# nilsbore/gp_compressor

Hardware: AMD Instinct MI355X
Metric: patches/sec (compress+predict) (higher is better)
Workload: dtype f64; 1 GPU; C2 room scan: 8192 patches x 256 pts per GPU, RBF + Gaussian noise, dense Cholesky fit + predictive mean on the 20x20 grid (m=400); patches_per_gpu=8192, points_per_patch=256, grid_points=400, parallelism=1 GPU, kernel=dense_mfma_w1

## Files before the change

### gp_compressor_amd/csrc/dense_mfma_w1.hip

```cpp
#include <cstdio>
#include <cstdlib>
#include <type_traits>

#include "gpc_device.h"
#include "dense_internal.h"
#include "mfma_tile.h"

#define W1_NPAD_MAX 512
#define W1_C 4
#define W1_NDT 10
#define W1_NT_OF(npad) ((npad) / 16)
#define W1_TRI_OF(npad) (W1_NT_OF(npad) * (W1_NT_OF(npad) + 1) / 2)
#define W1_TILE(i, j) (((size_t)(i) * (size_t)((i) + 1) / 2 + (size_t)(j)) * MF_IMG)


struct W1Params {
    DenseArgs a;
    double c_exp;
    double pivot_tol;
    double cs, noise_u, sfp, a_out;
    double* ws;
    double* linvt;
    int export_factor;
    unsigned long long* stamps;
};
#define W1_NPH 12
#ifdef W1_STAMPS
#define W1_STAMP(ph)                                                                                                 \
    do {                                                                                                             \
        __builtin_amdgcn_sched_barrier(0);                                                                           \
        const unsigned long long t_now_ = __builtin_amdgcn_s_memtime();                                              \
        st_acc_[ph] += t_now_ - t_prev_;                                                                             \
        t_prev_ = t_now_;                                                                                            \
        __builtin_amdgcn_sched_barrier(0);                                                                           \
    } while (0)
#else
#define W1_STAMP(ph) do { } while (0)
#endif

#define W1_LDS_SYNC()                                                                                                \
    do {                                                                                                             \
        __builtin_amdgcn_fence(__ATOMIC_SEQ_CST, "wavefront");                                                       \
        __builtin_amdgcn_wave_barrier();                                                                             \
    } while (0)

template <int A, int B, typename F>
__device__ static __forceinline__ void w1_static_for(F&& f)
{
    if constexpr (A < B) {
        f(std::integral_constant<int, A>{});
        w1_static_for<A + 1, B>(f);
    }
}
__host__ __device__ constexpr int w1_stream_col(int q)
{
    int kk = 0;
    while ((kk + 1) * (kk + 2) / 2 <= q) ++kk;
    return kk;
}
#define W1_BW 20

__device__ static __forceinline__ d4 w1_mfma4_neg(d4 a, d4 b, d4 acc)
{
#pragma unroll
    for (int s = 0; s < 4; ++s) acc = __builtin_amdgcn_mfma_f64_16x16x4f64(a[s], b[s], acc, 0, 0, 1);
    return acc;
}
__device__ static __forceinline__ d4 w1_trsm(d4 lv, d4 src)
{
    const d4 z4 = d4{0.0, 0.0, 0.0, 0.0};
    d4 D = __builtin_amdgcn_mfma_f64_16x16x4f64(lv[0], src[0], z4, 0, 0, 0);
    D = __builtin_amdgcn_mfma_f64_16x16x4f64(lv[1], src[1], D, 0, 0, 0);
    D = __builtin_amdgcn_mfma_f64_16x16x4f64(lv[2], src[2], D, 0, 0, 0);
    return __builtin_amdgcn_mfma_f64_16x16x4f64(lv[3], src[3], D, 0, 0, 0);
}

template <int MODE, int CNT, bool DIAG>
__device__ static __forceinline__ void w1_gram_row(d4 (&v)[W1_C], const double* px0, const double* px1, const double* T, double sf, bool scale_sf,
                                                   double cexp, double noise, bool dbl, int n, int r, int c0, int lr, int lg)
{
    const int pi = MF_TS * r + lr;
    const double xi0 = px0[pi], xi1 = px1[pi];
#pragma unroll
    for (int t = 0; t < CNT; ++t) {
#pragma unroll
        for (int q = 0; q < 4; ++q) {
            const int pj = MF_TS * (c0 + t) + lg + 4 * q;
            const double d0 = xi0 - px0[pj], d1 = xi1 - px1[pj];
            const double sq = __builtin_fma(d0, d0, d1 * d1);
            v[t][q] = MODE == 0 ? gpc_exp_neg(cexp * sq, T) : gpc_expm_poly<MODE == 1 ? 7 : 5>(sq);
        }
    }
    if (scale_sf) {
#pragma unroll
        for (int t = 0; t < CNT; ++t)
#pragma unroll
            for (int q = 0; q < 4; ++q) v[t][q] *= sf;
    }
    if constexpr (DIAG) {
#pragma unroll
        for (int q = 0; q < 4; ++q) {
            double d = v[CNT - 1][q] + noise;
            if (dbl) d += noise;
            v[CNT - 1][q] = (lr == lg + 4 * q) ? d : v[CNT - 1][q];
        }
    }
    if (MF_TS * (r + 1) > n || MF_TS * (c0 + CNT) > n) {
#pragma unroll
        for (int t = 0; t < CNT; ++t) {
#pragma unroll
            for (int q = 0; q < 4; ++q) {
                const int pj = MF_TS * (c0 + t) + lg + 4 * q;
                if (pi >= n || pj >= n) v[t][q] = (pi == pj) ? 1.0 : 0.0;
            }
        }
    }
}

template <int W1_NPAD>
__global__ __launch_bounds__(64, 2) void dense_w1_kernel(W1Params g)
{
    constexpr int W1_NT = W1_NT_OF(W1_NPAD), W1_TRI = W1_TRI_OF(W1_NPAD);
    __shared__ __attribute__((aligned(16))) double T[GPC_EXP_TABLE_SIZE];
    __shared__ __attribute__((aligned(16))) double px0[W1_NPAD], px1[W1_NPAD], zv[W1_NPAD];
    __shared__ __attribute__((aligned(16))) double rsbuf[32], wsc[32];
    __shared__ __attribute__((aligned(16))) double LinvC[W1_C * MF_IMG];

    const DenseArgs& A = g.a;
    int lane = threadIdx.x;
    int lr = lane & 15, lg = lane >> 4;
#define W1_FRESH_LANE()                                                                                              \
    do {                                                                                                             \
        lane = mf_opaque(lane);                                                                                      \
        lr = lane & 15;                                                                                              \
        lg = lane >> 4;                                                                                              \
    } while (0)
    const int m = A.m;
    const double sf = A.prm.sigmaf_sq, cexp = g.c_exp;
    const bool dbl = A.prm.ref_double_noise != 0;
    const int patch = blockIdx.x;
    double* Lt = g.ws + (size_t)patch * W1_TRI * MF_IMG;
    double* LinvTg = g.linvt + (size_t)patch * W1_NT * MF_IMG;

    gpc_exp_table_init(T);
    {
        const int o = __builtin_amdgcn_readfirstlane(A.off[patch]);
        const int n = __builtin_amdgcn_readfirstlane(A.off[patch + 1]) - o;
        double* fs = A.f_star + (size_t)patch * m;
        __syncthreads();
        if (n <= 0 || n > W1_NPAD) {
            for (int p = lane; p < m; p += 64) fs[p] = (n == 0) ? 0.0 : __builtin_nan("");
            if (lane == 0 && A.status) A.status[patch] = (n == 0) ? GPC_STATUS_OK : GPC_STATUS_NAN;
            return;
        }
        const int nt = __builtin_amdgcn_readfirstlane((n + MF_TS - 1) / MF_TS);
#ifdef W1_STAMPS
        unsigned long long st_acc_[W1_NPH] = {};
        unsigned long long t_prev_ = __builtin_amdgcn_s_memtime();
#endif

        const double xo0 = A.x0[o], xo1 = A.x1[o];
        double qr0[W1_NPAD / 64], qr1[W1_NPAD / 64];
        double mn0 = xo0, mx0 = xo0, mn1 = xo1, mx1 = xo1;
#pragma unroll
        for (int u = 0; u < W1_NPAD / 64; ++u) {
            const int i = lane + 64 * u;
            const bool live = i < n;
            qr0[u] = live ? A.x0[o + i] : xo0;
            qr1[u] = live ? A.x1[o + i] : xo1;
            mn0 = __builtin_fmin(mn0, qr0[u]); mx0 = __builtin_fmax(mx0, qr0[u]);
            mn1 = __builtin_fmin(mn1, qr1[u]); mx1 = __builtin_fmax(mx1, qr1[u]);
            zv[i] = live ? A.y[o + i] : 0.0;
        }
#pragma unroll
        for (int o_ = 32; o_ > 0; o_ >>= 1) {
            mn0 = __builtin_fmin(mn0, __shfl_xor(mn0, o_, 64)); mx0 = __builtin_fmax(mx0, __shfl_xor(mx0, o_, 64));
            mn1 = __builtin_fmin(mn1, __shfl_xor(mn1, o_, 64)); mx1 = __builtin_fmax(mx1, __shfl_xor(mx1, o_, 64));
        }
        int mode_g, mode_p;
        {
            const bool nan_box = !((mx0 - mn0) + (mx1 - mn1) < __builtin_inf());
            const double rx = mx0 - mn0, ry = mx1 - mn1;
            const double tg = nan_box ? __builtin_inf() : -cexp * __builtin_fma(rx, rx, ry * ry);
            const double hb = 0.5 * A.grid_res;
            const double bx = hb + __builtin_fmax(__builtin_fabs(mn0), __builtin_fabs(mx0));
            const double by = hb + __builtin_fmax(__builtin_fabs(mn1), __builtin_fabs(mx1));
            const double bq = __builtin_fmax(bx, by);
            const double tp = nan_box ? __builtin_inf() : -cexp * (bq * bq);
            mode_g = __builtin_amdgcn_readfirstlane(tg <= GPC_EXP_TINY_MAX ? 2 : tg <= GPC_EXP_SMALL_MAX ? 1 : 0);
            mode_p = __builtin_amdgcn_readfirstlane(tp <= GPC_EXP_TINY_MAX ? 2 : tp <= GPC_EXP_SMALL_MAX ? 1 : 0);
            if (mode_g == 0) mode_p = 0;
        }
        const bool scaled = mode_g > 0;
        {
            const double cs = scaled ? g.cs : 1.0;
            const double co0 = scaled ? xo0 : 0.0, co1 = scaled ? xo1 : 0.0;
#pragma unroll
            for (int u = 0; u < W1_NPAD / 64; ++u) {
                const int i = lane + 64 * u;
                const bool live = i < n;
                px0[i] = live ? cs * (qr0[u] - co0) : 0.0;
                px1[i] = live ? cs * (qr1[u] - co1) : 0.0;
            }
        }
        const bool scale_sf = g.export_factor != 0;
        const double noise_u = g.noise_u, ptol = g.pivot_tol;
        W1_LDS_SYNC();
#define W1_GRAM_ROW(v, CNT, DIAG, r, c0)                                                                              \
    do {                                                                                                             \
        if (mode_g == 2) w1_gram_row<2, CNT, DIAG>(v, px0, px1, T, sf, scale_sf, cexp, noise_u, dbl, n, r, c0, lr, lg);   \
        else if (mode_g == 1) w1_gram_row<1, CNT, DIAG>(v, px0, px1, T, sf, scale_sf, cexp, noise_u, dbl, n, r, c0, lr, lg); \
        else w1_gram_row<0, CNT, DIAG>(v, px0, px1, T, sf, scale_sf, cexp, noise_u, dbl, n, r, c0, lr, lg);            \
    } while (0)

        auto bw_step = [&](auto P, const d4 img, d4& pa) __attribute__((always_inline)) {
            constexpr int q = decltype(P)::value;
            constexpr int kk = w1_stream_col(q), t = q - kk * (kk + 1) / 2;
            if (kk < nt) {
                const int k = nt - 1 - kk;
                if constexpr (t < kk) {
                    const double a_ = zv[MF_TS * (k + 1 + t) + lr];
                    pa += img * a_;
                } else {
                    d4 ub = d4{0.0, 0.0, 0.0, 0.0};
                    if constexpr (kk > 0) {
                        const double tot = mf_row_reduce4(pa, lr);
                        if ((lr & 3) == 0) wsc[lg + 4 * (lr >> 2)] = tot;
                        W1_LDS_SYNC();
                        if (lr == 0) {
#pragma unroll
                            for (int q4 = 0; q4 < 4; ++q4) ub[q4] = zv[MF_TS * k + lg + 4 * q4] - wsc[lg + 4 * q4];
                        }
                    } else {
                        if (lr == 0) {
#pragma unroll
                            for (int q4 = 0; q4 < 4; ++q4) ub[q4] = zv[MF_TS * k + lg + 4 * q4];
                        }
                    }
                    const d4 al = w1_trsm(img, ub);
                    W1_LDS_SYNC();
                    if (lr == 0) {
#pragma unroll
                        for (int r = 0; r < 4; ++r) zv[MF_TS * k + lg + 4 * r] = al[r];
                    }
                    W1_LDS_SYNC();
                    pa = d4{0.0, 0.0, 0.0, 0.0};
                }
            }
        };
        bool bad = false;
        W1_STAMP(0);
#define W1_BLOCK_ROW(bi, kb, nb)                                                                                     \
    do {                                                                                                             \
        if ((bi) < (nb)) {                                                                                           \
            d4 gv[W1_C];                                                                                             \
            W1_GRAM_ROW(gv, (bi) + 1, true, (kb) + (bi), (kb));                                                      \
            _Pragma("unroll") for (int bc = 0; bc <= (bi); ++bc) tacc[(bi) * ((bi) + 1) / 2 + bc] = gv[bc];           \
        } else {                                                                                                     \
            _Pragma("unroll") for (int bc = 0; bc <= (bi); ++bc) tacc[(bi) * ((bi) + 1) / 2 + bc] = d4{0.0, 0.0, 0.0, 0.0}; \
        }                                                                                                            \
    } while (0)
#define W1_BLOCK_INIT(kb, nb)                                                                                        \
    do {                                                                                                             \
        _Pragma("unroll") for (int i = 0; i < W1_C; ++i) part[i] = 0.0;                                              \
                                             \
        __builtin_amdgcn_sched_barrier(0);                                                                           \
        W1_BLOCK_ROW(3, kb, nb);                                                                                     \
        __builtin_amdgcn_sched_barrier(0);                                                                           \
        W1_BLOCK_ROW(2, kb, nb);                                                                                     \
        __builtin_amdgcn_sched_barrier(0);                                                                           \
        W1_BLOCK_ROW(1, kb, nb);                                                                                     \
        __builtin_amdgcn_sched_barrier(0);                                                                           \
        W1_BLOCK_ROW(0, kb, nb);                                                                                     \
        __builtin_amdgcn_sched_barrier(0);                                                                           \
    } while (0)
        W1_STAMP(1);
        for (int k = 0;; k += W1_C) {
            const int nc = min(W1_C, nt - k);
            const int kl = k - 1;
            const bool last_step = k + W1_C >= nt;
            (void)last_step;
            W1_FRESH_LANE();
            const double* rrow[W1_C];
#pragma unroll
            for (int i = 0; i < W1_C; ++i) rrow[i] = Lt + W1_TILE(k + min(i, nc - 1), 0);
            d4 tacc[W1_NDT];
            double part[W1_C];
            d4 op[2][W1_C];
#pragma unroll
            for (int i = 0; i < W1_C; ++i) op[0][i] = op[1][i] = d4{0.0, 0.0, 0.0, 0.0};
            if (k > 0) {
#pragma unroll
                for (int i = 0; i < W1_C; ++i) op[0][i] = mf_img_load(rrow[i], lane);
            }
            W1_BLOCK_INIT(k, nc);
            for (int j = 0; j < k; j += 2) {
#pragma unroll
                for (int h = 0; h < 2; ++h) {
                    const int jn = min(j + h + 1, kl);
#pragma unroll
                    for (int i = 0; i < W1_C; ++i) op[h ^ 1][i] = mf_img_load(rrow[i] + (size_t)jn * MF_IMG, lane);
#pragma unroll
                    for (int d = 0; d < W1_NDT; ++d) {
                        const int bi = d >= 6 ? 3 : d >= 3 ? 2 : d >= 1 ? 1 : 0, bc = d - bi * (bi + 1) / 2;
                        if (bi < nc) tacc[d] = w1_mfma4_neg(op[h][bc], op[h][bi], tacc[d]);
                    }
                    const double* zq = zv + MF_TS * (j + h) + lg;
                    const double z0 = zq[0], z1 = zq[4], z2 = zq[8], z3 = zq[12];
#pragma unroll
                    for (int c = 0; c < W1_C; ++c) part[c] += (op[h][c][0] * z0 + op[h][c][1] * z1) + (op[h][c][2] * z2 + op[h][c][3] * z3);
                }
            }
            W1_STAMP(2);
            W1_FRESH_LANE();
            d4 Lb[W1_C * (W1_C - 1) / 2];
#pragma unroll
            for (int q = 0; q < W1_C * (W1_C - 1) / 2; ++q) Lb[q] = d4{0.0, 0.0, 0.0, 0.0};
            bool ok = mf_diag_factor_c(tacc[0], rsbuf, LinvC, LinvTg + (size_t)k * MF_IMG, ptol, lane);
            W1_LDS_SYNC();
            if (g.export_factor) mf_img_store(Lt + W1_TILE(k, k), lane, mf_img_load(LinvC, lane));
#pragma unroll
            for (int i = 1; i < W1_C; ++i) {
                if (ok && i < nc) {
#pragma unroll
                    for (int c = 0; c < i; ++c) {
                        d4 Tt = tacc[i * (i + 1) / 2 + c];
#pragma unroll
                        for (int c2 = 0; c2 < c; ++c2) Tt = w1_mfma4_neg(Lb[c * (c - 1) / 2 + c2], Lb[i * (i - 1) / 2 + c2], Tt);
                        const d4 lvc = mf_img_load(LinvC + c * MF_IMG, mf_opaque(lane));
                        const d4 L = w1_trsm(lvc, Tt);
                        Lb[i * (i - 1) / 2 + c] = L;
                        mf_img_store(Lt + W1_TILE(k + i, k + c), lane, L);
                    }
                    d4 Dii = tacc[i * (i + 1) / 2 + i];
#pragma unroll
                    for (int c = 0; c < i; ++c) Dii = w1_mfma4_neg(Lb[i * (i - 1) / 2 + c], Lb[i * (i - 1) / 2 + c], Dii);
                    ok = mf_diag_factor_c(Dii, rsbuf, LinvC + i * MF_IMG, LinvTg + (size_t)(k + i) * MF_IMG, ptol, lane);
                    W1_LDS_SYNC();
                    if (g.export_factor) mf_img_store(Lt + W1_TILE(k + i, k + i), lane, mf_img_load(LinvC + i * MF_IMG, mf_opaque(lane)));
                }
            }
            if (!ok) { bad = true; break; }
            W1_STAMP(3);
            W1_FRESH_LANE();
#pragma unroll
            for (int c = 0; c < W1_C; ++c) {
                if (c < nc) {
                    const int pj = MF_TS * (k + c) + lr;
                    double pp = part[c];
#pragma unroll
                    for (int c2 = 0; c2 < c; ++c2) {
                        const d4 lb = Lb[c * (c - 1) / 2 + c2];
                        const double* zq = zv + MF_TS * (k + c2) + lg;
                        pp += (lb[0] * zq[0] + lb[1] * zq[4]) + (lb[2] * zq[8] + lb[3] * zq[12]);
                    }
                    pp += __shfl_xor(pp, 16, 64);
                    pp += __shfl_xor(pp, 32, 64);
                    const double yv = zv[pj];
                    W1_LDS_SYNC();
                    if (lg == 0) zv[pj] = yv - pp;
                    W1_LDS_SYNC();
                    const d4 lv = mf_img_load(LinvC + c * MF_IMG, mf_opaque(lane));
                    const double* tq = zv + MF_TS * (k + c) + lg;
                    double zz = (lv[0] * tq[0] + lv[1] * tq[4]) + (lv[2] * tq[8] + lv[3] * tq[12]);
                    zz += __shfl_xor(zz, 16, 64);
                    zz += __shfl_xor(zz, 32, 64);
                    W1_LDS_SYNC();
                    if (lg == 0) zv[pj] = zz;
                    W1_LDS_SYNC();
                }
            }
            W1_STAMP(4);
            const int rows_tot = nt - (k + nc);
            if (rows_tot == 0) {
                __syncthreads();
                break;
            }
            if (k > 0) __syncthreads();
            const int npass = (rows_tot + 3) / 4;
            const int klp = k - 1;
            if (k == 0) {
                for (int pi_ = 0; pi_ < npass; ++pi_) {
                    const int first_row0 = (pi_ + 1 < npass) ? 4 * (pi_ + 1) : 0;
                    const int np4 = min(4, rows_tot - first_row0);
                    W1_FRESH_LANE();
                    d4 cy[W1_C][4];
#pragma unroll
                    for (int t = 0; t < 4; ++t) {
                        const int r_ = W1_C + first_row0 + min(t, np4 - 1);
                        d4 gv[W1_C];
                        W1_GRAM_ROW(gv, 2, false, r_, 0);
                        cy[0][t] = gv[0]; cy[1][t] = gv[1];
                        __builtin_amdgcn_sched_barrier(0);
                        W1_GRAM_ROW(gv, 2, false, r_, 2);
                        cy[2][t] = gv[0]; cy[3][t] = gv[1];
                        __builtin_amdgcn_sched_barrier(0);
                    }
                    W1_STAMP(5);
#pragma unroll
                    for (int c = 0; c < W1_C; ++c) {
                        const d4 lv = mf_img_load(LinvC + c * MF_IMG, mf_opaque(lane));
#pragma unroll
                        for (int t = 0; t < 4; ++t) {
#pragma unroll
                            for (int c2 = 0; c2 < c; ++c2) cy[c][t] = w1_mfma4_neg(Lb[c * (c - 1) / 2 + c2], cy[c2][t], cy[c][t]);
                            cy[c][t] = w1_trsm(lv, cy[c][t]);
                            if (t < np4) mf_img_store(Lt + W1_TILE(W1_C + first_row0 + t, c), lane, cy[c][t]);
                        }
                    }
                    W1_STAMP(7);
                }
            }
            if (k > 0) {
                for (int pi_ = 0; pi_ < npass; ++pi_) {
                    const int first_row = (pi_ + 1 < npass) ? 4 * (pi_ + 1) : 0;
                    const int np4 = min(4, rows_tot - first_row);
                    W1_FRESH_LANE();
                    d4 cy[W1_C][4];
                    int rr[4];
                    const double* rw_[4];
#pragma unroll
                    for (int t = 0; t < 4; ++t) {
                        rr[t] = k + W1_C + first_row + min(t, np4 - 1);
                        rw_[t] = Lt + W1_TILE(rr[t], 0);
                    }
                    d4 A2[2][W1_C], B[4];
#pragma unroll
                    for (int c = 0; c < W1_C; ++c) A2[0][c] = mf_img_load(rrow[c], lane);
#pragma unroll
                    for (int t = 0; t < 4; ++t) B[t] = mf_img_load(rw_[t], lane);
#pragma unroll
                    for (int t = 0; t < 4; ++t) {
                        d4 gv[W1_C];
                        W1_GRAM_ROW(gv, 2, false, rr[t], k);
                        cy[0][t] = gv[0]; cy[1][t] = gv[1];
                        __builtin_amdgcn_sched_barrier(0);
                        W1_GRAM_ROW(gv, 2, false, rr[t], k + 2);
                        cy[2][t] = gv[0]; cy[3][t] = gv[1];
                        __builtin_amdgcn_sched_barrier(0);
                    }
                    W1_STAMP(5);
                    d4 Lq[W1_C * (W1_C - 1) / 2];
#define W1_PASS_J(st, jn, PREFETCH)                                                                                  \
    do {                                                                                                             \
                                      \
        if (PREFETCH) {                                                                                              \
            _Pragma("unroll") for (int c = 0; c < W1_C; ++c) A2[(st) ^ 1][c] = mf_img_load(rrow[c] + (size_t)(jn) * MF_IMG, lane); \
        }                                                                                                            \
        __builtin_amdgcn_sched_barrier(0);                                                                           \
        _Pragma("unroll") for (int t = 0; t < 4; ++t) {                                                              \
            _Pragma("unroll") for (int c = 0; c < W1_C; ++c) cy[c][t] = w1_mfma4_neg(A2[st][c], B[t], cy[c][t]);      \
            __builtin_amdgcn_sched_barrier(0);                                                                       \
            if (PREFETCH) B[t] = mf_img_load(rw_[t] + (size_t)(jn) * MF_IMG, lane);                                    \
            else {      \
                if (t < 3) Lq[t] = mf_img_load(Lt + W1_TILE(k + (t == 0 ? 1 : 2), k + (t == 2 ? 1 : 0)), lane);      \
                else {                                                                                               \
                    _Pragma("unroll") for (int c2 = 0; c2 < 3; ++c2) Lq[3 + c2] = mf_img_load(Lt + W1_TILE(k + 3, k + c2), lane); \
                }                                                                                                    \
            }                                                                                                        \
            __builtin_amdgcn_sched_barrier(0);                                                                       \
        }                                                                                                            \
    } while (0)
                    for (int j = 0; j + 2 < k; j += 2) {
                        W1_PASS_J(0, j + 1, true);
                        W1_PASS_J(1, j + 2, true);
                    }
                    W1_PASS_J(0, klp, true);
                    W1_PASS_J(1, klp, false);
#undef W1_PASS_J
                    W1_STAMP(6);
                    W1_FRESH_LANE();
#pragma unroll
                    for (int c = 0; c < W1_C; ++c) {
                        const d4 lv = mf_img_load(LinvC + c * MF_IMG, mf_opaque(lane));
#pragma unroll
                        for (int t = 0; t < 4; ++t) {
#pragma unroll
                            for (int c2 = 0; c2 < c; ++c2) cy[c][t] = w1_mfma4_neg(Lq[c * (c - 1) / 2 + c2], cy[c2][t], cy[c][t]);
                            cy[c][t] = w1_trsm(lv, cy[c][t]);
                            if (t < np4) mf_img_store(Lt + W1_TILE(rr[t], k + c), lane, cy[c][t]);
                        }
                    }
                    W1_STAMP(7);
                }
            }
            __syncthreads();
            W1_STAMP(8);
        }
#undef W1_BLOCK_INIT
#undef W1_BLOCK_ROW

        if (bad) {
            for (int p = lane; p < m; p += 64) fs[p] = __builtin_nan("");
            if (A.alpha_out)
                for (int i = lane; i < n; i += 64) A.alpha_out[o + i] = __builtin_nan("");
            if (lane == 0 && A.status) A.status[patch] = GPC_STATUS_NOT_SPD;
            return;
        }

        {
            W1_FRESH_LANE();
            constexpr int NP = W1_NPAD / MF_TS;
            constexpr int SLEN = NP * (NP + 1) / 2;
            d4 win[W1_BW];
            auto stream_addr = [&](auto P) __attribute__((always_inline)) -> const double* {
                constexpr int q = decltype(P)::value;
                constexpr int kk = w1_stream_col(q), t = q - kk * (kk + 1) / 2;
                const int kq = max(nt - 1 - kk, 0);
                const double* ad = (t < kk) ? Lt + W1_TILE(kq + 1 + t, kq) : LinvTg + (size_t)kq * MF_IMG;
                return kk < nt ? ad : Lt;
            };
            w1_static_for<0, W1_BW>([&](auto P) __attribute__((always_inline)) {
                constexpr int q = decltype(P)::value;
                win[q] = mf_img_load_nt(stream_addr(P), lane);
            });
            d4 pa = d4{0.0, 0.0, 0.0, 0.0};
            w1_static_for<0, SLEN>([&](auto P) __attribute__((always_inline)) {
                constexpr int q = decltype(P)::value;
                bw_step(P, win[q % W1_BW], pa);
                if constexpr (q + W1_BW < SLEN) {
                    win[q % W1_BW] = mf_img_load_nt(stream_addr(std::integral_constant<int, q + W1_BW>{}), lane);
                }
            });
        }
        W1_STAMP(9);
        double* av = zv;
        if (A.alpha_out)
            for (int i = lane; i < n; i += 64) A.alpha_out[o + i] = av[i] * g.a_out;

        W1_FRESH_LANE();
        if (m <= 0) {
        } else if (A.xs0 == nullptr && A.grid_sz <= 32) {
            const int sz = A.grid_sz;
            const double res = A.grid_res;
            d4 P[2][2];
#pragma unroll
            for (int mt = 0; mt < 2; ++mt)
#pragma unroll
                for (int nl = 0; nl < 2; ++nl) P[mt][nl] = d4{0.0, 0.0, 0.0, 0.0};
            double gqx[2], gqy[2];
            const double cs = scaled ? g.cs : 1.0, co0 = scaled ? A.x0[o] : 0.0, co1 = scaled ? A.x1[o] : 0.0;
            const double argc = scaled ? -1.0 : cexp, sfp = g.sfp;
#pragma unroll
            for (int h = 0; h < 2; ++h) {
                const double gq = res * (((double)(16 * h + lr) + 0.5) / (double)sz - 0.5);
                gqx[h] = cs * (gq - co0);
                gqy[h] = cs * (gq - co1);
            }
            auto predict_loop = [&](auto mode_tag) __attribute__((always_inline)) {
                constexpr int MP = decltype(mode_tag)::value;
                for (int ibase = 0; ibase < n; ibase += 32) {
#pragma unroll
                    for (int s = 0; s < 8; ++s) {
                        const int i = ibase + 4 * s + lg;
                        const int ic = min(i, W1_NPAD - 1);
                        const double al = (i < n) ? sfp * av[ic] : 0.0;
                        const double xi0 = px0[ic], xi1 = px1[ic];
                        double ea[2], eb[2];
#pragma unroll
                        for (int h = 0; h < 2; ++h) {
                            const double dy = gqy[h] - xi1, dx = gqx[h] - xi0;
                            if constexpr (MP == 0) {
                                ea[h] = gpc_exp_neg(argc * (dy * dy), T);
                                eb[h] = gpc_exp_neg(argc * (dx * dx), T) * al;
                            } else {
                                ea[h] = gpc_expm_poly<MP == 1 ? 7 : 5>(dy * dy);
                                eb[h] = gpc_expm_poly<MP == 1 ? 7 : 5>(dx * dx) * al;
                            }
                        }
#pragma unroll
                        for (int nl = 0; nl < 2; ++nl)
#pragma unroll
                            for (int mt = 0; mt < 2; ++mt)
                                P[mt][nl] = __builtin_amdgcn_mfma_f64_16x16x4f64(ea[mt], eb[nl], P[mt][nl], 0, 0, 0);
                    }
                }
            };
            if (mode_p == 2) predict_loop(std::integral_constant<int, 2>{});
            else if (mode_p == 1) predict_loop(std::integral_constant<int, 1>{});
            else predict_loop(std::integral_constant<int, 0>{});
#pragma unroll
            for (int mt = 0; mt < 2; ++mt)
#pragma unroll
                for (int nl = 0; nl < 2; ++nl)
#pragma unroll
                    for (int r = 0; r < 4; ++r) {
                        const int py = 16 * mt + lg + 4 * r, pxx = 16 * nl + lr;
                        if (py < sz && pxx < sz) fs[py * sz + pxx] = P[mt][nl][r];
                    }
        } else {
            const double cs = scaled ? g.cs : 1.0, co0 = scaled ? A.x0[o] : 0.0, co1 = scaled ? A.x1[o] : 0.0;
            const double argc = scaled ? -1.0 : cexp, sfp = g.sfp;
            for (int p = lane; p < m; p += 64) {
                double q0, q1;
                if (A.xs0) {
                    q0 = A.xs0[p];
                    q1 = A.xs1[p];
                } else {
                    const int gx = p % A.grid_sz, gy = p / A.grid_sz;
                    q0 = A.grid_res * (((double)gx + 0.5) / (double)A.grid_sz - 0.5);
                    q1 = A.grid_res * (((double)gy + 0.5) / (double)A.grid_sz - 0.5);
                }
                q0 = cs * (q0 - co0);
                q1 = cs * (q1 - co1);
                double s_ = 0.0;
                for (int i = 0; i < n; ++i) {
                    const double d0 = px0[i] - q0, d1 = px1[i] - q1;
                    s_ += gpc_exp_neg(argc * __builtin_fma(d0, d0, d1 * d1), T) * av[i];
                }
                fs[p] = sfp * s_;
            }
        }
        if (lane == 0 && A.status) A.status[patch] = GPC_STATUS_OK;
#ifdef W1_STAMPS
        W1_STAMP(10);
        if (g.stamps && lane == 0)
            for (int q_ = 0; q_ < W1_NPH; ++q_) atomicAdd(g.stamps + q_, st_acc_[q_]);
#endif
    }
}

static int w1_npad(const DenseArgs& a) { return a.n_max <= 256 ? 256 : W1_NPAD_MAX; }

bool dense_w1_supported(const DenseArgs& a)
{
    if (a.v_star) return a.n_max <= 256 && a.ny == 1 && !a.sel && a.xs0 != nullptr;
    return a.n_max <= W1_NPAD_MAX && a.ny == 1 && !a.sel;
}

#define W1_MAX_SLOTS 8192
static int w1_chunk(const DenseArgs& a, int cap_in)
{
    const char* e = getenv("GPC_W1_SLOTS");
    int cap = e && atoi(e) > 0 ? atoi(e) : W1_MAX_SLOTS;
    if (cap_in > 0 && cap_in < cap) cap = cap_in;
    return a.P < cap ? a.P : cap;
}

size_t dense_w1_ws_bytes(const gpc_ctx* ctx, const DenseArgs& a, int* grid_out, int cap)
{
    (void)ctx;
    const int grid = w1_chunk(a, cap);
    if (grid_out) *grid_out = grid;
    const int npad = w1_npad(a);
    return sizeof(double) * ((size_t)(W1_TRI_OF(npad) + W1_NT_OF(npad)) * MF_IMG * (size_t)grid + (a.v_star ? (size_t)a.n_total : 0));
}

int dense_w1_launch(gpc_ctx* ctx, const DenseSite& site, const DenseArgs& a_in, int grid)
{
    DenseArgs a = a_in;
    double* v_star = a.v_star;
    a.v_star = nullptr;
    W1Params g;
    g.c_exp = (double)(-0.5f) / a.prm.l_sq;
    g.ws = reinterpret_cast<double*>(dense_ws(ctx, site));
    const int npad = w1_npad(a);
    g.linvt = g.ws + (size_t)W1_TRI_OF(npad) * MF_IMG * (size_t)grid;
    g.export_factor = v_star ? 1 : 0;
    const double sf = a.prm.sigmaf_sq;
    const bool unit = !v_star;
    g.cs = sqrt(-g.c_exp);
    g.noise_u = unit ? a.prm.noise / sf : a.prm.noise;
    g.pivot_tol = GPC_PIVOT_RTOL * (unit ? 1.0 + a.prm.noise / sf : sf + a.prm.noise);
    g.sfp = unit ? 1.0 : sf;
    g.a_out = unit ? 1.0 / sf : 1.0;
    g.stamps = nullptr;
    if (v_star) {
        a.m = 0;
        if (!a.alpha_out) a.alpha_out = g.linvt + (size_t)W1_NT_OF(npad) * MF_IMG * (size_t)grid;
    }
    ctx->last_dense_kernel = v_star ? "dense_mfma_w1 + dense_variance" : npad == 256 ? "dense_mfma_w1" : "dense_mfma_w1_512";
#ifdef W1_STAMPS
    if (getenv("GPC_W1_STAMPS")) {
        GPC_HIP(ctx, hipMalloc(&g.stamps, sizeof(unsigned long long) * W1_NPH));
        GPC_HIP(ctx, hipMemsetAsync(g.stamps, 0, sizeof(unsigned long long) * W1_NPH, site.stream));
    }
#endif
    for (int base = 0; base < a.P; base += grid) {
        const int cnt = a.P - base < grid ? a.P - base : grid;
        g.a = a;
        g.a.P = cnt;
        g.a.off = a.off + base;
        g.a.f_star = a.f_star ? a.f_star + (size_t)base * a.ny * a_in.m : nullptr;
        g.a.status = a.status ? a.status + base : nullptr;
        if (npad == 256) hipLaunchKernelGGL((dense_w1_kernel<256>), dim3(cnt), dim3(64), 0, site.stream, g);
        else hipLaunchKernelGGL((dense_w1_kernel<W1_NPAD_MAX>), dim3(cnt), dim3(64), 0, site.stream, g);
        GPC_HIP(ctx, hipGetLastError());
        if (v_star) {
            DenseArgs av = g.a;
            av.m = a_in.m;
            const int rc = dense_variance_launch(ctx, site, av, W1_NT_OF(256), g.ws, a.alpha_out, v_star + (size_t)base * a_in.m);
            if (rc != GPC_OK) return rc;
        }
    }
#ifdef W1_STAMPS
    if (g.stamps) {
        unsigned long long h[W1_NPH];
        GPC_HIP(ctx, hipStreamSynchronize(site.stream));
        GPC_HIP(ctx, hipMemcpy(h, g.stamps, sizeof(h), hipMemcpyDeviceToHost));
        (void)hipFree(g.stamps);
        static const char* names[W1_NPH] = {"load", "sweep gram", "sweep loop", "chain", "forward", "pass gram", "pass loop", "pass trsm",
                                            "step fence", "backward", "predict", ""};
        unsigned long long tot = 0;
        for (int q = 0; q < W1_NPH; ++q) tot += h[q];
        fprintf(stderr, "[GPC_W1_STAMPS] mean s_memtime ticks per patch (total %.0f)\n", (double)tot / a.P);
        for (int q = 0; q < 11; ++q) fprintf(stderr, "  %-12s %9.0f  %5.1f %%\n", names[q], (double)h[q] / a.P, 100.0 * h[q] / tot);
    }
#endif
    return GPC_OK;
}
```

### gp_compressor_amd/csrc/mfma_tile.h

```cpp
#pragma once

#include "gpc_device.h"

typedef double d4 __attribute__((ext_vector_type(4)));
#define MF_TS 16

__device__ static __forceinline__ int mf_opaque(int v)
{
    asm volatile("" : "+v"(v));
    return v;
}

__device__ static __forceinline__ bool mf_wait_ge(unsigned lds_byte_addr, int k)
{
    int v, cnt;
    asm volatile(
        "s_mov_b32 %1, 0x100000\n\t"
        "1:\n\t"
        "ds_read_b32 %0, %2\n\t"
        "s_waitcnt lgkmcnt(0)\n\t"
        "v_cmp_gt_i32 vcc, %3, %0\n\t"
        "s_cbranch_vccz 2f\n\t"
        "s_sub_u32 %1, %1, 1\n\t"
        "s_cmp_eq_u32 %1, 0\n\t"
        "s_cbranch_scc1 2f\n\t"
        "s_sleep 1\n\t"
        "s_branch 1b\n\t"
        "2:\n\t"
        : "=&v"(v), "=&s"(cnt)
        : "v"(lds_byte_addr), "v"(k)
        : "vcc", "scc", "memory");
    return cnt != 0;
}
__device__ static __forceinline__ void mf_publish(int* word, int k)
{
    __hip_atomic_store(word, k, __ATOMIC_RELEASE, __HIP_MEMORY_SCOPE_WORKGROUP);
}

__device__ static __forceinline__ double mf_readlane(double v, int lane_const)
{
    const int lo = __builtin_amdgcn_readlane(__double2loint(v), lane_const);
    const int hi = __builtin_amdgcn_readlane(__double2hiint(v), lane_const);
    return __hiloint2double(hi, lo);
}

__device__ static __forceinline__ double mf_rsqrt(double d)
{
    double y = __builtin_amdgcn_rsq(d);
    double e = __builtin_fma(-d * y, y, 1.0);
    y = __builtin_fma(y * 0.5, e, y);
    e = __builtin_fma(-d * y, y, 1.0);
    y = __builtin_fma(y * 0.5, e, y);
    return y;
}
__device__ static __forceinline__ double mf_rcp(double d)
{
    double y = __builtin_amdgcn_rcp(d);
    double e = __builtin_fma(-d, y, 1.0);
    y = __builtin_fma(y, e, y);
    e = __builtin_fma(-d, y, 1.0);
    y = __builtin_fma(y, e, y);
    return y;
}

typedef double d2 __attribute__((ext_vector_type(2)));
#define MF_IMG 256
__device__ static __forceinline__ int mf_img_off(int l, int s) { return (s >> 1) * 128 + l * 2 + (s & 1); }
__device__ static __forceinline__ int mf_img_rc(int r, int c) { return mf_img_off(r + 16 * (c & 3), c >> 2); }
__device__ static __forceinline__ d4 mf_img_load(const double* img, int l)
{
    const d2 a = *reinterpret_cast<const d2*>(img + l * 2);
    const d2 b = *reinterpret_cast<const d2*>(img + 128 + l * 2);
    return d4{a[0], a[1], b[0], b[1]};
}
__device__ static __forceinline__ void mf_img_store(double* img, int l, d4 v)
{
    *reinterpret_cast<d2*>(img + l * 2) = d2{v[0], v[1]};
    *reinterpret_cast<d2*>(img + 128 + l * 2) = d2{v[2], v[3]};
}

__device__ static __forceinline__ d4 mf_img_load_nt(const double* img, int l)
{
    const d2 a = __builtin_nontemporal_load(reinterpret_cast<const d2*>(img + l * 2));
    const d2 b = __builtin_nontemporal_load(reinterpret_cast<const d2*>(img + 128 + l * 2));
    return d4{a[0], a[1], b[0], b[1]};
}
__device__ static __forceinline__ void mf_img_store_nt(double* img, int l, d4 v)
{
    __builtin_nontemporal_store(d2{v[0], v[1]}, reinterpret_cast<d2*>(img + l * 2));
    __builtin_nontemporal_store(d2{v[2], v[3]}, reinterpret_cast<d2*>(img + 128 + l * 2));
}

template <bool OPAQUE = false>
__device__ __forceinline__ static bool mf_diag_factor(d4 W, double* rsbuf, double* Linv_out, double* LinvT_out, double pivot_tol, int lane_in = -1)
{
    const int lane = OPAQUE ? mf_opaque(lane_in >= 0 ? lane_in : (int)(threadIdx.x & 63)) : (int)(threadIdx.x & 63);
    const int lr = lane & 15, lg = lane >> 4;
    double rp = mf_rcp(mf_readlane(W[0], 0));
    double rpv = (lg == 0 && lr > 0) ? rp : 0.0;
    double one_q = (lg == 0) ? 1.0 : 0.0, ev = (lane == 0) ? 1.0 : 0.0;
#pragma unroll
    for (int c = 0; c < MF_TS - 1; ++c) {
        const int q = c & 3, r = c >> 2, q1 = (c + 1) & 3, r1 = (c + 1) >> 2;
        if constexpr (!OPAQUE) {
            one_q = (lg == q) ? 1.0 : 0.0;
            ev = (lg == q && lr == c) ? 1.0 : 0.0;
        }
        const double a_op = W[r] * rpv;
        const double b_op = __builtin_fma(W[r], one_q, ev);
        const d4 Wn = __builtin_amdgcn_mfma_f64_16x16x4f64(a_op, b_op, W, 0, 0, 1);
        __builtin_amdgcn_sched_barrier(0);
        const double s01 = mf_readlane(W[r], 16 * q + c + 1);
        const double s11 = mf_readlane(W[r1], 16 * q1 + c + 1);
        const double t = s01 * rp;
        rp = mf_rcp(__builtin_fma(-t, s01, s11));
        if constexpr (OPAQUE) {
            const int lo_ = mf_opaque(lane);
            const int lr_ = lo_ & 15, lg_ = lo_ >> 4;
            rpv = (lg_ == q1 && lr_ > c + 1) ? rp : 0.0;
            one_q = (lg_ == q1) ? 1.0 : 0.0;
            ev = (lo_ == 16 * q1 + c + 1) ? 1.0 : 0.0;
        } else {
            rpv = (lg == q1 && lr > c + 1) ? rp : 0.0;
        }
        __builtin_amdgcn_sched_barrier(0);
        W = Wn;
    }
    const int lt_ = OPAQUE ? mf_opaque(lane) : lane;
    const int lrt = lt_ & 15, lgt = lt_ >> 4;
    const int rsel = lrt >> 2;
    const double pd = rsel == 0 ? W[0] : rsel == 1 ? W[1] : rsel == 2 ? W[2] : W[3];
    const bool on_diag = (lrt & 3) == lgt;
    const bool ok = __builtin_amdgcn_ballot_w64(on_diag && !(pd > pivot_tol)) == 0;
    const double rs = mf_rsqrt(on_diag ? pd : 1.0);
    if (on_diag) rsbuf[lrt] = rs;
    d4 fin;
#pragma unroll
    for (int r = 0; r < 4; ++r) {
        const int row = lgt + 4 * r;
        const double rsr = rsbuf[row];
        fin[r] = (lrt < row) ? W[r] * rsr : (lrt == row ? rsr : 0.0);
    }
    mf_img_store(LinvT_out, lt_, fin);
#pragma unroll
    for (int r = 0; r < 4; ++r) Linv_out[mf_img_rc(lgt + 4 * r, lrt)] = fin[r];
    return ok;
}

__device__ static __forceinline__ int mf_sel32(int v, unsigned long long mask)
{
    int r;
    asm("v_cndmask_b32_e64 %0, 0, %1, %2" : "=v"(r) : "v"(v), "s"(mask));
    return r;
}
__device__ static __forceinline__ double mf_sel64(double v, unsigned long long mask)
{
    return __hiloint2double(mf_sel32(__double2hiint(v), mask), mf_sel32(__double2loint(v), mask));
}
__device__ static __forceinline__ double mf_one_in(unsigned long long mask, int one_hi)
{
    return __hiloint2double(mf_sel32(one_hi, mask), 0);
}
__device__ __forceinline__ static bool mf_diag_factor_c(d4 W, double* rsbuf, double* Linv_out, double* LinvT_out, double pivot_tol, int lane_in)
{
    const int one_hi = 0x3FF00000;
    double rp = mf_rcp(mf_readlane(W[0], 0));
    double rpv = mf_sel64(rp, 0xFFFEull);
    double one_q = mf_one_in(0xFFFFull, one_hi);
    double ev = mf_one_in(0x1ull, one_hi);
#pragma unroll
    for (int c = 0; c < MF_TS - 1; ++c) {
        const int q = c & 3, r = c >> 2, q1 = (c + 1) & 3, r1 = (c + 1) >> 2;
        const double a_op = W[r] * rpv;
        const double b_op = __builtin_fma(W[r], one_q, ev);
        const d4 Wn = __builtin_amdgcn_mfma_f64_16x16x4f64(a_op, b_op, W, 0, 0, 1);
        __builtin_amdgcn_sched_barrier(0);
        const double s01 = mf_readlane(W[r], 16 * q + c + 1);
        const double s11 = mf_readlane(W[r1], 16 * q1 + c + 1);
        const double t = s01 * rp;
        rp = mf_rcp(__builtin_fma(-t, s01, s11));
        const unsigned long long slot = 0xFFFFull << (16 * q1);
        const unsigned long long below = ((0xFFFFull << (c + 2)) & 0xFFFFull) << (16 * q1);
        rpv = mf_sel64(rp, below);
        one_q = mf_one_in(slot, one_hi);
        ev = mf_one_in(1ull << (16 * q1 + c + 1), one_hi);
        __builtin_amdgcn_sched_barrier(0);
        W = Wn;
    }
    const int lt_ = mf_opaque(lane_in);
    const int lrt = lt_ & 15, lgt = lt_ >> 4;
    const int rsel = lrt >> 2;
    const double pd = rsel == 0 ? W[0] : rsel == 1 ? W[1] : rsel == 2 ? W[2] : W[3];
    const bool on_diag = (lrt & 3) == lgt;
    const bool ok = __builtin_amdgcn_ballot_w64(on_diag && !(pd > pivot_tol)) == 0;
    const double rs = mf_rsqrt(on_diag ? pd : 1.0);
    if (on_diag) rsbuf[lrt] = rs;
    d4 fin;
#pragma unroll
    for (int r = 0; r < 4; ++r) {
        const int row = lgt + 4 * r;
        const double rsr = rsbuf[row];
        fin[r] = (lrt < row) ? W[r] * rsr : (lrt == row ? rsr : 0.0);
    }
    if (LinvT_out) mf_img_store(LinvT_out, lt_, fin);
#pragma unroll
    for (int r = 0; r < 4; ++r) Linv_out[mf_img_rc(lgt + 4 * r, lrt)] = fin[r];
    return ok;
}

__device__ static __forceinline__ double mf_row_dot(const double* img, int mr, const double* v)
{
    double s_ = 0.0;
#pragma unroll
    for (int gq = 0; gq < 4; ++gq) {
        const d4 ch = mf_img_load(img, mr + 16 * gq);
#pragma unroll
        for (int s = 0; s < 4; ++s) s_ = __builtin_fma(ch[s], v[gq + 4 * s], s_);
    }
    return s_;
}

template <int CTRL>
__device__ static __forceinline__ double mf_dpp(double v)
{
    const int lo = __builtin_amdgcn_mov_dpp(__double2loint(v), CTRL, 0xf, 0xf, true);
    const int hi = __builtin_amdgcn_mov_dpp(__double2hiint(v), CTRL, 0xf, 0xf, true);
    return __hiloint2double(hi, lo);
}
__device__ static __forceinline__ double mf_row_allsum(double v)
{
    v += mf_dpp<0x121>(v);
    v += mf_dpp<0x122>(v);
    v += mf_dpp<0x124>(v);
    v += mf_dpp<0x128>(v);
    return v;
}

__device__ static __forceinline__ double mf_row_reduce4(d4 x, int lr)
{
    const bool hi8 = (lr & 8) != 0, hi4 = (lr & 4) != 0;
    double k0 = hi8 ? x[2] : x[0], k1 = hi8 ? x[3] : x[1];
    const double s0 = hi8 ? x[0] : x[2], s1 = hi8 ? x[1] : x[3];
    k0 += mf_dpp<0x128>(s0);
    k1 += mf_dpp<0x128>(s1);
    double k = hi4 ? k1 : k0;
    const double sd = hi4 ? k0 : k1;
    k += mf_dpp<0x141>(sd);
    k += mf_dpp<0xB1>(k);
    k += mf_dpp<0x4E>(k);
    return k;
}
```

Before: 5.548 million patches/s.

## Pack pairs of triangular inverse diagonal tiles into one global tile

For npad<=256, two consecutive triangular inverse diagonal tiles (one transposed, one reversed) are packed into a single 16x16 tile, with the overlapping diagonal kept in LDS. This halves the LinvT workspace and the global traffic for it. The backward substitution stream is rewritten to unpack these tiles with mask selects and to solve the second block in reversed order. It adds select instructions, extra LDS syncs and more complex index logic.

```diff
diff --git a/gp_compressor_amd/csrc/dense_mfma_w1.hip b/gp_compressor_amd/csrc/dense_mfma_w1.hip
--- a/gp_compressor_amd/csrc/dense_mfma_w1.hip
+++ b/gp_compressor_amd/csrc/dense_mfma_w1.hip
@@ -12,6 +12,8 @@
 #define W1_NT_OF(npad) ((npad) / 16)
 #define W1_TRI_OF(npad) (W1_NT_OF(npad) * (W1_NT_OF(npad) + 1) / 2)
 #define W1_TILE(i, j) (((size_t)(i) * (size_t)((i) + 1) / 2 + (size_t)(j)) * MF_IMG)
+#define W1_PACK_OF(npad) ((npad) <= 256)
+#define W1_LNV_OF(npad) (W1_PACK_OF(npad) ? W1_NT_OF(npad) / 2 : W1_NT_OF(npad))
 
 
 struct W1Params {
@@ -58,6 +60,12 @@
     while ((kk + 1) * (kk + 2) / 2 <= q) ++kk;
     return kk;
 }
+__host__ __device__ constexpr int w1_pstream_pair(int q)
+{
+    int pp = 0;
+    while (2 * (pp + 1) * (pp + 1) <= q) ++pp;
+    return pp;
+}
 #define W1_BW 20
 
 __device__ static __forceinline__ d4 w1_mfma4_neg(d4 a, d4 b, d4 acc)
@@ -125,6 +133,9 @@
     __shared__ __attribute__((aligned(16))) double px0[W1_NPAD], px1[W1_NPAD], zv[W1_NPAD];
     __shared__ __attribute__((aligned(16))) double rsbuf[32], wsc[32];
     __shared__ __attribute__((aligned(16))) double LinvC[W1_C * MF_IMG];
+    constexpr bool W1_PACK = W1_PACK_OF(W1_NPAD);
+    constexpr int W1_LNV = W1_LNV_OF(W1_NPAD);
+    __shared__ __attribute__((aligned(16))) double dgl[W1_PACK ? W1_LNV * MF_TS : 2];
 
     const DenseArgs& A = g.a;
     int lane = threadIdx.x;
@@ -140,7 +151,7 @@
     const bool dbl = A.prm.ref_double_noise != 0;
     const int patch = blockIdx.x;
     double* Lt = g.ws + (size_t)patch * W1_TRI * MF_IMG;
-    double* LinvTg = g.linvt + (size_t)patch * W1_NT * MF_IMG;
+    double* LinvTg = g.linvt + (size_t)patch * W1_LNV * MF_IMG;
 
     gpc_exp_table_init(T);
     {
@@ -213,6 +224,30 @@
         else w1_gram_row<0, CNT, DIAG>(v, px0, px1, T, sf, scale_sf, cexp, noise_u, dbl, n, r, c0, lr, lg);            \
     } while (0)
 
+        auto bw_close = [&](auto HASW, auto REV, const int k, const d4 img, d4& pa) __attribute__((always_inline)) {
+            constexpr bool has_w = decltype(HASW)::value, rev = decltype(REV)::value;
+            d4 ub = d4{0.0, 0.0, 0.0, 0.0};
+            if constexpr (has_w) {
+                const double tot = mf_row_reduce4(pa, lr);
+                if ((lr & 3) == 0) wsc[lg + 4 * (lr >> 2)] = tot;
+                W1_LDS_SYNC();
+            }
+            if (lr == 0) {
+#pragma unroll
+                for (int q4 = 0; q4 < 4; ++q4) {
+                    const int e = rev ? MF_TS - 1 - (lg + 4 * q4) : lg + 4 * q4;
+                    ub[q4] = has_w ? zv[MF_TS * k + e] - wsc[e] : zv[MF_TS * k + e];
+                }
+            }
+            const d4 al = w1_trsm(img, ub);
+            W1_LDS_SYNC();
+            if (lr == 0) {
+#pragma unroll
+                for (int r = 0; r < 4; ++r) zv[MF_TS * k + (rev ? MF_TS - 1 - (lg + 4 * r) : lg + 4 * r)] = al[r];
+            }
+            W1_LDS_SYNC();
+            pa = d4{0.0, 0.0, 0.0, 0.0};
+        };
         auto bw_step = [&](auto P, const d4 img, d4& pa) __attribute__((always_inline)) {
             constexpr int q = decltype(P)::value;
             constexpr int kk = w1_stream_col(q), t = q - kk * (kk + 1) / 2;
@@ -222,29 +257,7 @@
                     const double a_ = zv[MF_TS * (k + 1 + t) + lr];
                     pa += img * a_;
                 } else {
-                    d4 ub = d4{0.0, 0.0, 0.0, 0.0};
-                    if constexpr (kk > 0) {
-                        const double tot = mf_row_reduce4(pa, lr);
-                        if ((lr & 3) == 0) wsc[lg + 4 * (lr >> 2)] = tot;
-                        W1_LDS_SYNC();
-                        if (lr == 0) {
-#pragma unroll
-                            for (int q4 = 0; q4 < 4; ++q4) ub[q4] = zv[MF_TS * k + lg + 4 * q4] - wsc[lg + 4 * q4];
-                        }
-                    } else {
-                        if (lr == 0) {
-#pragma unroll
-                            for (int q4 = 0; q4 < 4; ++q4) ub[q4] = zv[MF_TS * k + lg + 4 * q4];
-                        }
-                    }
-                    const d4 al = w1_trsm(img, ub);
-                    W1_LDS_SYNC();
-                    if (lr == 0) {
-#pragma unroll
-                        for (int r = 0; r < 4; ++r) zv[MF_TS * k + lg + 4 * r] = al[r];
-                    }
-                    W1_LDS_SYNC();
-                    pa = d4{0.0, 0.0, 0.0, 0.0};
+                    bw_close(std::bool_constant<(kk > 0)>{}, std::false_type{}, k, img, pa);
                 }
             }
         };
@@ -279,7 +292,6 @@
             const int nc = min(W1_C, nt - k);
             const int kl = k - 1;
             const bool last_step = k + W1_C >= nt;
-            (void)last_step;
             W1_FRESH_LANE();
             const double* rrow[W1_C];
 #pragma unroll
@@ -316,7 +328,7 @@
             d4 Lb[W1_C * (W1_C - 1) / 2];
 #pragma unroll
             for (int q = 0; q < W1_C * (W1_C - 1) / 2; ++q) Lb[q] = d4{0.0, 0.0, 0.0, 0.0};
-            bool ok = mf_diag_factor_c(tacc[0], rsbuf, LinvC, LinvTg + (size_t)k * MF_IMG, ptol, lane);
+            bool ok = mf_diag_factor_c(tacc[0], rsbuf, LinvC, W1_PACK ? nullptr : LinvTg + (size_t)k * MF_IMG, ptol, lane);
             W1_LDS_SYNC();
             if (g.export_factor) mf_img_store(Lt + W1_TILE(k, k), lane, mf_img_load(LinvC, lane));
 #pragma unroll
@@ -335,12 +347,24 @@
                     d4 Dii = tacc[i * (i + 1) / 2 + i];
 #pragma unroll
                     for (int c = 0; c < i; ++c) Dii = w1_mfma4_neg(Lb[i * (i - 1) / 2 + c], Lb[i * (i - 1) / 2 + c], Dii);
-                    ok = mf_diag_factor_c(Dii, rsbuf, LinvC + i * MF_IMG, LinvTg + (size_t)(k + i) * MF_IMG, ptol, lane);
+                    ok = mf_diag_factor_c(Dii, rsbuf, LinvC + i * MF_IMG, W1_PACK ? nullptr : LinvTg + (size_t)(k + i) * MF_IMG, ptol, lane);
                     W1_LDS_SYNC();
                     if (g.export_factor) mf_img_store(Lt + W1_TILE(k + i, k + i), lane, mf_img_load(LinvC + i * MF_IMG, mf_opaque(lane)));
                 }
             }
             if (!ok) { bad = true; break; }
+            if constexpr (W1_PACK) {
+                if (!last_step) {
+#pragma unroll
+                    for (int h = 0; h < 2; ++h) {
+                        const int lp = mf_opaque(lane), pr = (k >> 1) + h;
+                        const double* Lo = LinvC + (2 * h + 1) * MF_IMG;
+                        const d4 pk = mf_tri_pack(mf_img_load_t(LinvC + 2 * h * MF_IMG, lp), mf_img_load_tr(Lo, lp));
+                        mf_img_store(LinvTg + (size_t)pr * MF_IMG, lp, pk);
+                        if (lp < MF_TS) dgl[MF_TS * pr + lp] = Lo[mf_img_rc(MF_TS - 1 - lp, MF_TS - 1 - lp)];
+                    }
+                }
+            }
             W1_STAMP(3);
             W1_FRESH_LANE();
 #pragma unroll
@@ -498,7 +522,71 @@
             return;
         }
 
-        {
+        if constexpr (W1_PACK) {
+            W1_FRESH_LANE();
+            constexpr int NP = W1_NT;
+            constexpr int SLEN = NP * NP / 2;
+            const int nte = (nt + 1) & ~1, kls = (nt - 1) & ~(W1_C - 1);
+            d4 win[W1_BW];
+            auto stream_addr = [&](auto P) __attribute__((always_inline)) -> const double* {
+                constexpr int q = decltype(P)::value;
+                constexpr int pp = w1_pstream_pair(q), i = q - 2 * pp * pp;
+                if constexpr (i == 2 * pp) {
+                    const int k = nte - 1 - 2 * pp;
+                    return (k >= 1 && k - 1 < kls) ? LinvTg + (size_t)(k >> 1) * MF_IMG : Lt;
+                } else {
+                    constexpr int kk = i < 2 * pp ? 2 * pp : 2 * pp + 1, t = i < 2 * pp ? i : i - 2 * pp - 1;
+                    const int k = nte - 1 - kk, kq = max(k, 0);
+                    return (k >= 0 && k + 1 + t < nt) ? Lt + W1_TILE(kq + 1 + t, kq) : Lt;
+                }
+            };
+            w1_static_for<0, W1_BW>([&](auto P) __attribute__((always_inline)) {
+                constexpr int q = decltype(P)::value;
+                win[q] = mf_img_load_nt(stream_addr(P), lane);
+            });
+            d4 pa = d4{0.0, 0.0, 0.0, 0.0};
+            double* const held = LinvC + (W1_C - 1) * MF_IMG;
+            w1_static_for<0, SLEN>([&](auto P) __attribute__((always_inline)) {
+                constexpr int q = decltype(P)::value;
+                constexpr int pp = w1_pstream_pair(q), i = q - 2 * pp * pp;
+                const d4 img = win[q % W1_BW];
+                if constexpr (i == 2 * pp) {
+                    const int k = nte - 1 - 2 * pp;
+                    if (k >= 1) {
+                        d4 lo;
+                        bool in_lds = false;
+                        if constexpr (pp < W1_C / 2) in_lds = k - 1 >= kls;
+                        if (in_lds) {
+                            const double* Lc = LinvC + (k - 1 - kls) * MF_IMG;
+                            lo = mf_img_load_tr(Lc + MF_IMG, lane);
+                        } else {
+                            mf_img_store(held, lane, mf_tri_upper(img));
+                            lo = mf_tri_lower(img, dgl[MF_TS * (k >> 1) + lr]);
+                            W1_LDS_SYNC();
+                        }
+                        if (k < nt) bw_close(std::bool_constant<(pp > 0)>{}, std::true_type{}, k, lo, pa);
+                    }
+                } else {
+                    constexpr int kk = i < 2 * pp ? 2 * pp : 2 * pp + 1, t = i < 2 * pp ? i : i - 2 * pp - 1;
+                    const int k = nte - 1 - kk;
+                    if (k >= 0 && k + 1 + t < nt) {
+                        const double a_ = zv[MF_TS * (k + 1 + t) + lr];
+                        pa += img * a_;
+                    }
+                    if constexpr (i == 4 * pp + 1) {
+                        if (k >= 0) {
+                            bool in_lds = false;
+                            if constexpr (pp < W1_C / 2) in_lds = k >= kls;
+                            const d4 up = in_lds ? mf_img_load_t(LinvC + (k - kls) * MF_IMG, lane) : mf_img_load(held, lane);
+                            bw_close(std::true_type{}, std::false_type{}, k, up, pa);
+                        }
+                    }
+                }
+                if constexpr (q + W1_BW < SLEN) {
+                    win[q % W1_BW] = mf_img_load_nt(stream_addr(std::integral_constant<int, q + W1_BW>{}), lane);
+                }
+            });
+        } else {
             W1_FRESH_LANE();
             constexpr int NP = W1_NPAD / MF_TS;
             constexpr int SLEN = NP * (NP + 1) / 2;
@@ -643,7 +731,7 @@
     const int grid = w1_chunk(a, cap);
     if (grid_out) *grid_out = grid;
     const int npad = w1_npad(a);
-    return sizeof(double) * ((size_t)(W1_TRI_OF(npad) + W1_NT_OF(npad)) * MF_IMG * (size_t)grid + (a.v_star ? (size_t)a.n_total : 0));
+    return sizeof(double) * ((size_t)(W1_TRI_OF(npad) + W1_LNV_OF(npad)) * MF_IMG * (size_t)grid + (a.v_star ? (size_t)a.n_total : 0));
 }
 
 int dense_w1_launch(gpc_ctx* ctx, const DenseSite& site, const DenseArgs& a_in, int grid)
@@ -667,7 +755,7 @@
     g.stamps = nullptr;
     if (v_star) {
         a.m = 0;
-        if (!a.alpha_out) a.alpha_out = g.linvt + (size_t)W1_NT_OF(npad) * MF_IMG * (size_t)grid;
+        if (!a.alpha_out) a.alpha_out = g.linvt + (size_t)W1_LNV_OF(npad) * MF_IMG * (size_t)grid;
     }
     ctx->last_dense_kernel = v_star ? "dense_mfma_w1 + dense_variance" : npad == 256 ? "dense_mfma_w1" : "dense_mfma_w1_512";
 #ifdef W1_STAMPS
diff --git a/gp_compressor_amd/csrc/mfma_tile.h b/gp_compressor_amd/csrc/mfma_tile.h
--- a/gp_compressor_amd/csrc/mfma_tile.h
+++ b/gp_compressor_amd/csrc/mfma_tile.h
@@ -208,6 +208,53 @@
     return ok;
 }
 
+__host__ __device__ constexpr unsigned long long mf_tri_mask(int s, int kind)
+{
+    unsigned long long m = 0;
+    for (int l = 0; l < 64; ++l) {
+        const int r = l & 15, c = (l >> 4) + 4 * s;
+        if (kind == 0 ? r <= c : kind == 1 ? r == c : r > c) m |= 1ull << l;
+    }
+    return m;
+}
+__device__ static __forceinline__ int mf_mix32(int a, int b, unsigned long long mask)
+{
+    int r;
+    asm("v_cndmask_b32_e64 %0, %1, %2, %3" : "=v"(r) : "v"(b), "v"(a), "s"(mask));
+    return r;
+}
+__device__ static __forceinline__ double mf_mix64(double a, double b, unsigned long long mask)
+{
+    return __hiloint2double(mf_mix32(__double2hiint(a), __double2hiint(b), mask), mf_mix32(__double2loint(a), __double2loint(b), mask));
+}
+__device__ static __forceinline__ d4 mf_tri_pack(d4 up, d4 lo)
+{
+    constexpr unsigned long long u0 = mf_tri_mask(0, 0), u1 = mf_tri_mask(1, 0), u2 = mf_tri_mask(2, 0), u3 = mf_tri_mask(3, 0);
+    return d4{mf_mix64(up[0], lo[0], u0), mf_mix64(up[1], lo[1], u1), mf_mix64(up[2], lo[2], u2), mf_mix64(up[3], lo[3], u3)};
+}
+__device__ static __forceinline__ d4 mf_tri_upper(d4 p)
+{
+    constexpr unsigned long long u0 = mf_tri_mask(0, 0), u1 = mf_tri_mask(1, 0), u2 = mf_tri_mask(2, 0), u3 = mf_tri_mask(3, 0);
+    return d4{mf_sel64(p[0], u0), mf_sel64(p[1], u1), mf_sel64(p[2], u2), mf_sel64(p[3], u3)};
+}
+__device__ static __forceinline__ d4 mf_tri_lower(d4 p, double dg)
+{
+    constexpr unsigned long long l0 = mf_tri_mask(0, 2), l1 = mf_tri_mask(1, 2), l2 = mf_tri_mask(2, 2), l3 = mf_tri_mask(3, 2);
+    constexpr unsigned long long e0 = mf_tri_mask(0, 1), e1 = mf_tri_mask(1, 1), e2 = mf_tri_mask(2, 1), e3 = mf_tri_mask(3, 1);
+    return d4{mf_mix64(dg, mf_sel64(p[0], l0), e0), mf_mix64(dg, mf_sel64(p[1], l1), e1), mf_mix64(dg, mf_sel64(p[2], l2), e2),
+              mf_mix64(dg, mf_sel64(p[3], l3), e3)};
+}
+__device__ static __forceinline__ d4 mf_img_load_t(const double* img, int l)
+{
+    const int lr = l & 15, lg = l >> 4;
+    return d4{img[mf_img_rc(lg, lr)], img[mf_img_rc(lg + 4, lr)], img[mf_img_rc(lg + 8, lr)], img[mf_img_rc(lg + 12, lr)]};
+}
+__device__ static __forceinline__ d4 mf_img_load_tr(const double* img, int l)
+{
+    const int lr = 15 - (l & 15), lg = 15 - (l >> 4);
+    return d4{img[mf_img_rc(lg, lr)], img[mf_img_rc(lg - 4, lr)], img[mf_img_rc(lg - 8, lr)], img[mf_img_rc(lg - 12, lr)]};
+}
+
 __device__ static __forceinline__ double mf_row_dot(const double* img, int mr, const double* v)
 {
     double s_ = 0.0;
```

Result: faster. 5.605 million patches/s (median of 6 runs) (+1.0%).
